# askerlee/segtran

Measured on AMD Instinct MI355X. Metric: train-step images/sec (cfg2, re-associated op order), higher is better.
Workload: dtype f32; 1 GPU; REFUGE fundus 2D, segtran eff-b4, translayers 3, layercompress 1,1,2,2, 512x512, bs 6/GPU; global_batch=6, per_gpu_batch=6, parallelism=dp1, step=fwd+BCE/Dice+bwd+allreduce+clip+BertAdam, op_order=re-associated, ranks=1

## Files before the change

include/segx.h:

```cpp
#ifndef SEGX_H
#define SEGX_H
#include <stdint.h>
#ifdef __cplusplus
extern "C" {
#endif

int segx_version(void);
int segx_last_error(char* buf, int buflen);

enum { SEGX_EPI_NONE = 0, SEGX_EPI_GELU = 1 ,
       SEGX_EPI_SWISH = 2 ,
       SEGX_EPI_RELU = 3  };
enum { SEGX_BIAS_NONE = 0, SEGX_BIAS_N = 1 , SEGX_BIAS_M = 2  };
enum { SEGX_ENGINE_F32 = 0, SEGX_ENGINE_BF16X6 = 1 };
enum { SEGX_ENGINE_SEL_DEFAULT = 0, SEGX_ENGINE_SEL_F32 = 1, SEGX_ENGINE_SEL_BF16X6 = 2 };
enum { SEGX_TILE_AUTO = 0, SEGX_TILE_128x128 = 1, SEGX_TILE_64x64 = 2, SEGX_TILE_128x32 = 3, SEGX_TILE_32x128 = 4, SEGX_TILE_64x128 = 5,
       SEGX_TILE_256x128 = 6, SEGX_TILE_WS128x128 = 7, SEGX_TILE_WS128x256 = 8, SEGX_TILE_WS64x256 = 9,
       SEGX_TILE_WS96x256 = 10, SEGX_TILE_WS256x96 = 11,
       SEGX_TILE_SKINNY_NT = 12   };
typedef struct {
    int32_t M, N, K, nb0, nb1;
    int64_t a_b0, a_b1, a_m, a_k;
    int64_t b_b0, b_b1, b_n, b_k;
    int64_t c_b0, c_b1, c_m;
// ... 163 lines not shown
int segx_set_rng_base(const uint64_t* base);
int segx_rng_advance(uint64_t* base, uint64_t span, void* stream);

enum {
    SEGX_KNOB_INTERP_VARIANT = 1,
    SEGX_KNOB_CONV_SMALL_POLICY = 2,
    SEGX_KNOB_BN_PATH = 3,
    SEGX_KNOB_ENGINE = 4,
    SEGX_KNOB_X6_LAUNCHES = 5,
    SEGX_KNOB_X6_VARIANT = 6,
    SEGX_KNOB_CONV_X6_WGRAD_ALL = 7,
    SEGX_KNOB_DW_STRIP_OUTPUTS = 8,
    SEGX_KNOB_WS_GRID = 9,
    SEGX_KNOB_TEAM_SPIN = 12,
    SEGX_KNOB_TEAM_DROP = 13,
    SEGX_KNOB_POOL_SLAB = 14,
    SEGX_KNOB_POOL_DSLIDE = 15,
    SEGX_KNOB_CONV_HALO = 16,
    SEGX_KNOB_CONV_HALO_MIN_TILES = 17,
    SEGX_KNOB_SKINNY_NT = 18,
    SEGX_KNOB_TILE_WALK = 19
};
#define SEGX_KNOB_X6_TERMS 20
int segx_tune(int knob, int value);
int segx_tune_get(int knob);
int segx_x3_launches(void);
int segx_interp_linear_fwd_axis2(const float* in, const float* base, float* out, int64_t outer, int n1_in, int n1_out, int n2_in, int n2_out,
                                 int64_t inner, void* stream);
int segx_interp_linear_bwd_axis2(const float* dout, float* din, int64_t outer, int n1_out, int n1_in, int n2_out, int n2_in, int64_t inner, void* stream);
int segx_interp_linear_fwd(const float* in, const float* base, float* out, int64_t planes, int d, int h, int w, int D, int H, int W,
                           void* stream);
int segx_interp_linear_fwd_axis(const float* in, const float* base, float* out, int64_t outer, int n_in, int n_out, int64_t inner,
                                float src_scale, void* stream);
int segx_resized_crop3d(const float* X, float* Y, int64_t planes, const int* geom, void* stream);
int segx_interp_linear_bwd(const float* dout, float* din, int64_t planes, int d, int h, int w, int D, int H, int W, void* stream);
int segx_axis_gather(const float* X, float* Y, int64_t planes, const int* geom, void* stream);
int segx_pixel_shuffle2(const float* X, float* Y, int64_t planes, int h, int w, int inverse, void* stream);
int segx_add_noise(const float* X, const float* noise, float* Y, int64_t n, float mu, float sigma, int nonzero_only, uint64_t seed, uint64_t offset,
                   void* stream);
int segx_resize2d(const float* X, float* Y, int64_t planes, int h, int w, int H, int W, int mode, int quantize, void* stream);
int segx_color_blend(const float* X, float* Y, int B, int64_t HW, int mode, const float* factor, const float* pivot, int quantize, void* stream);
int64_t segx_gray_mean_ws_floats(int B, int64_t HW);
int segx_gray_mean(const float* X, float* mean, float* ws, int B, int64_t HW, int quantize, void* stream);
int segx_normalize(const float* X, float* Y, int B, int C, int64_t HW, float scale, const float* mean, const float* std, void* stream);

int segx_interp_linear_bwd_axis(const float* dout, float* din, int64_t outer, int n_out, int n_in, int64_t inner, float src_scale,
// ... 91 lines not shown
```

segtran_amd/csrc/common.h:

```cpp
#pragma once
#include <hip/hip_runtime.h>
#include <stdint.h>
#include <stdio.h>
#include <stdarg.h>
#include <string.h>
#include <math.h>
#include <atomic>
#include "../../include/segx.h"

typedef float f32x16 __attribute__((ext_vector_type(16)));
typedef float f32x4 __attribute__((ext_vector_type(4)));

namespace segx {

inline char* err_buf() { static thread_local char buf[512] = {0}; return buf; }
inline int fail(int code, const char* fmt, ...) {
    va_list ap; va_start(ap, fmt); vsnprintf(err_buf(), 512, fmt, ap); va_end(ap); return code;
}
inline int check_launch(const char* what) {
    hipError_t e = hipGetLastError();
    if (e != hipSuccess) return fail((int)e, "%s: %s", what, hipGetErrorString(e));
    return 0;
}
#ifndef SEGX_MIN_WAVES_PER_SIMD
// ... 200 lines not shown
__device__ __forceinline__ float gelu_erf_grad(float x) {
    const float cdf = 0.5f * (1.0f + erff(x * 0.70710678118654752440f));
    const float pdf = 0.39894228040143267794f * __expf(-0.5f * x * x);
    return cdf + x * pdf;
}

#define SEGX_KNOB_TABLE(X)                                                                                                                                        \
    X(1, interp_variant, 0, 0, 2)                                                                  \
    X(2, conv_small_policy, 0, 0, 1)                          \
    X(3, bn_path, 0, 0, 2)                            \
    X(4, engine, SEGX_ENGINE_F32, SEGX_ENGINE_F32, SEGX_ENGINE_BF16X6)                                                                   \
    X(6, x6_variant, 0, 0, 7)                                      \
    X(7, conv_x6_wgrad_all, 0, 0, 2)                  \
    X(8, dw_strip_outputs, 8192, 256, 2147483647)                                                         \
    X(9, ws_grid, 256, 8, 4096)                                                                         \
    X(12, team_spin, (int)TEAM_SPIN_LIMIT, 32, 1 << 24)                                                     \
    X(13, team_drop, 0, 0, 4096)                      \
    X(14, pool_slab, 0, 0, 2)                         \
    X(15, pool_dslide, 1, 0, 1)                       \
    X(16, conv_halo, 1, 0, 1)                         \
    X(17, conv_halo_min_tiles, 256, 1, 1 << 24)         \
    X(18, skinny_nt, 1, 0, 1)                         \
    X(19, tile_walk, 1, 0, 1)                         \
    X(20, x6_terms, 6, 3, 6)
struct Knobs {
#define SEGX_KNOB_FIELD(id, field, def, lo, hi) std::atomic<int> field{def};
    SEGX_KNOB_TABLE(SEGX_KNOB_FIELD)
#undef SEGX_KNOB_FIELD
    std::atomic<int> x6_launches{0};
    std::atomic<int> x3_launches{0};
};
inline Knobs& knobs() { static Knobs k; return k; }
inline int kget(const std::atomic<int>& a) { return a.load(std::memory_order_relaxed); }
int halo_fwd_terms();

inline const uint64_t*& rng_base() { static const uint64_t* p = nullptr; return p; }

inline int ceil_div(int64_t a, int64_t b) { return (int)((a + b - 1) / b); }
__device__ __forceinline__ unsigned xcd_block(unsigned b, unsigned n) {
    const unsigned q = n >> 3, r = n & 7, xcd = b & 7, idx = b >> 3;
    return (xcd < r ? xcd * (q + 1) : r * (q + 1) + (xcd - r) * q) + idx;
}
__host__ __device__ inline int64_t i64min(int64_t a, int64_t b) { return a < b ? a : b; }
__host__ __device__ inline int64_t i64max(int64_t a, int64_t b) { return a > b ? a : b; }

struct FastDiv { unsigned d, magic; };
__host__ __device__ inline FastDiv make_fastdiv(int d) { FastDiv f; f.d = (unsigned)d; f.magic = d <= 1 ? 0u : (unsigned)(((1ull << 32) + d - 1) / d); return f; }
// ... 9 lines not shown
```

segtran_amd/csrc/mbconv_mid.hip:

```cpp
#include "common.h"
#include <initializer_list>

namespace segx {

constexpr int MID_BMAX = 6;

template <int NT> __device__ __forceinline__ void mid_guards(f32x4* pl, int H, int W4) {
    for (int r = threadIdx.x; r <= H; r += NT) pl[r * (W4 + 1)] = f32x4{0.f, 0.f, 0.f, 0.f};
}
__device__ __forceinline__ void mid_window(float (&e)[12], const f32x4* pl, int p, int r, int dr, int H, int W4) {
    const bool rok = (unsigned)(r + dr) < (unsigned)H;
    const f32x4* q = pl + (rok ? p + dr * (W4 + 1) : p);
    const f32x4 a = q[-1], m = q[0], z = q[1];
    e[0] = rok ? a.x : 0.f; e[1] = rok ? a.y : 0.f; e[2] = rok ? a.z : 0.f; e[3] = rok ? a.w : 0.f;
    e[4] = rok ? m.x : 0.f; e[5] = rok ? m.y : 0.f; e[6] = rok ? m.z : 0.f; e[7] = rok ? m.w : 0.f;
    e[8] = rok ? z.x : 0.f; e[9] = rok ? z.y : 0.f; e[10] = rok ? z.z : 0.f; e[11] = rok ? z.w : 0.f;
}
template <int NW, int KP>
__device__ __forceinline__ void mid_stats(f32x4 (&v)[MID_BMAX][KP], int B, float n, float* red, float& m, float& q) {
    float s = 0.f;
#pragma unroll
    for (int b = 0; b < MID_BMAX; ++b)
#pragma unroll
        for (int k = 0; k < KP; ++k) {
            if (b >= B) v[b][k] = f32x4{0.f, 0.f, 0.f, 0.f};
            s += (v[b][k].x + v[b][k].y) + (v[b][k].z + v[b][k].w);
        }
    m = block_sum<NW>(s, red) / n;
    q = 0.f;
#pragma unroll
    for (int b = 0; b < MID_BMAX; ++b)
#pragma unroll
        for (int k = 0; k < KP; ++k) {
            const float d0 = v[b][k].x - m, d1 = v[b][k].y - m, d2 = v[b][k].z - m, d3 = v[b][k].w - m;
            q += b < B ? (d0 * d0 + d1 * d1) + (d2 * d2 + d3 * d3) : 0.f;
        }
    q = block_sum<NW>(q, red);
}
__device__ __forceinline__ void mid_running(float* run_mean, float* run_var, int c, float momentum, float m, float q, float n) {
    if (run_mean) {
        run_mean[c] = (1.0f - momentum) * run_mean[c] + momentum * m;
        run_var[c] = (1.0f - momentum) * run_var[c] + momentum * (q / fmaxf(n - 1.0f, 1.0f));
    }
}

struct MidFwdArgs {
    const float* E; const float* w0; const float* b0; float* rm0; float* rv0; const float* Wdw; const float* w1; const float* b1; float* rm1; float* rv1;
    float* D; float* Y; float* psum; float* mean0; float* var0; float* mean1; float* var1;
    float mom0, eps0, mom1, eps1; int C, H, W4;
};
template <int KP, int K>
__global__ __launch_bounds__(256) SEGX_MIN_WAVES_PER_SIMD(KP == 1 ? 4 : 2) void mbconv_mid_fwd_kernel(MidFwdArgs g, int B) {
    constexpr int NT = 256, P = K / 2, S4 = NT * KP;
    __shared__ float red[4];
    __shared__ f32x4 plane[2 * S4 + 1];
    const int tl = threadIdx.x, c = blockIdx.x, C = g.C, H = g.H, W4 = g.W4;
    constexpr int64_t S = 4 * S4;
    unsigned off[KP]; int row[KP], pos[KP];
#pragma unroll
    for (int k = 0; k < KP; ++k) { const int j = tl + NT * k; off[k] = 16u * (unsigned)j; row[k] = j / W4; pos[k] = j + row[k] + 1; }
    mid_guards<NT>(plane, H, W4);
    f32x4 v[MID_BMAX][KP];
#pragma unroll
    for (int b = 0; b < MID_BMAX; ++b) {
        const ws_gptr xb = ws_uniform_base(g.E + ((int64_t)(b < B ? b : 0) * C + c) * S);
#pragma unroll
        for (int k = 0; k < KP; ++k) v[b][k] = ws_load<f32x4>(xb, off[k]);
    }
    __builtin_amdgcn_sched_barrier(0);
    float w[K * K];
#pragma unroll
    for (int i = 0; i < K * K; ++i) w[i] = g.Wdw[(int64_t)c * K * K + i];
    const float n = (float)B * (float)S;
    float m, q;
    mid_stats<4, KP>(v, B, n, red, m, q);
    float var = q / n;
    if (tl == 0) { g.mean0[c] = m; g.var0[c] = var; mid_running(g.rm0, g.rv0, c, g.mom0, m, q, n); }
    const float sc0 = rsqrtf(var + g.eps0) * g.w0[c], sh0 = g.b0[c] - m * sc0;
#pragma unroll
    for (int b = 0; b < MID_BMAX; ++b) {
        if (b >= B) break;
#pragma unroll
        for (int k = 0; k < KP; ++k) {
            f32x4 o;
            o.x = act_fwd(v[b][k].x * sc0 + sh0, ACT_SWISH); o.y = act_fwd(v[b][k].y * sc0 + sh0, ACT_SWISH);
            o.z = act_fwd(v[b][k].z * sc0 + sh0, ACT_SWISH); o.w = act_fwd(v[b][k].w * sc0 + sh0, ACT_SWISH);
            plane[pos[k]] = o;
        }
        __syncthreads();
        const ws_gptr_w db = ws_uniform_base_w(g.D + ((int64_t)b * C + c) * S);
#pragma unroll
        for (int k = 0; k < KP; ++k) {
            float acc[4] = {0.f, 0.f, 0.f, 0.f};
#pragma unroll
            for (int ky = 0; ky < K; ++ky) {
                float e[12];
                mid_window(e, plane, pos[k], row[k], ky - P, H, W4);
#pragma unroll
                for (int j = 0; j < 4; ++j)
#pragma unroll
                    for (int kx = 0; kx < K; ++kx) acc[j] += w[ky * K + kx] * e[4 + j + kx - P];
#pragma unroll
                for (int j = 0; j < 4; ++j) SEGX_PIN(acc[j]);
            }
            v[b][k] = f32x4{acc[0], acc[1], acc[2], acc[3]};
            ws_store<f32x4>(db, off[k], v[b][k]);
        }
        __syncthreads();
        __builtin_amdgcn_sched_barrier(0);
    }
    mid_stats<4, KP>(v, B, n, red, m, q);
    var = q / n;
    if (tl == 0) { g.mean1[c] = m; g.var1[c] = var; mid_running(g.rm1, g.rv1, c, g.mom1, m, q, n); }
    const float sc1 = rsqrtf(var + g.eps1) * g.w1[c], sh1 = g.b1[c] - m * sc1;
#pragma unroll
    for (int b = 0; b < MID_BMAX; ++b) {
        if (b >= B) break;
        const ws_gptr_w yb = ws_uniform_base_w(g.Y + ((int64_t)b * C + c) * S);
        float acc = 0.f;
#pragma unroll
        for (int k = 0; k < KP; ++k) {
            f32x4 o;
            o.x = act_fwd(v[b][k].x * sc1 + sh1, ACT_SWISH); o.y = act_fwd(v[b][k].y * sc1 + sh1, ACT_SWISH);
            o.z = act_fwd(v[b][k].z * sc1 + sh1, ACT_SWISH); o.w = act_fwd(v[b][k].w * sc1 + sh1, ACT_SWISH);
            ws_store<f32x4>(yb, off[k], o);
            acc += (o.x + o.y) + (o.z + o.w);
        }
        acc = block_sum<4>(acc, red);
        if (tl == 0) g.psum[(int64_t)b * C + c] = acc;
        __builtin_amdgcn_sched_barrier(0);
    }
}

__device__ __forceinline__ double wave_sum_d(double v) {
#pragma unroll
    for (int o = 32; o > 0; o >>= 1) v += __shfl_xor(v, o);
    return v;
}
template <int NW> __device__ __forceinline__ double block_sum_d(double v, double* red) {
    v = wave_sum_d(v);
    __syncthreads();
    if ((threadIdx.x & 63) == 0) red[threadIdx.x >> 6] = v;
    __syncthreads();
    double s = 0.0;
#pragma unroll
    for (int i = 0; i < NW; ++i) s += red[i];
    return s;
}

struct MidBwdArgs {
    const float* dY; const float* dpool; const float* D; const float* E;
    const float* mean0; const float* var0; const float* mean1; const float* var1;
    const float* w0; const float* b0; const float* w1; const float* b1; const float* Wdw;
    float* dE; float* dw0; float* db0; float* dw1; float* db1; float* dWdw;
    float inv_S, eps0, eps1; int C, H, W4;
};
template <int NT, int KP, int K, bool HL>
__global__ __launch_bounds__(NT) void mbconv_mid_bwd_kernel(MidBwdArgs g, int B) {
    constexpr int NW = NT / 64, P = K / 2, S4 = NT * KP, KK = K * K;
    __shared__ double red[NW];
    __shared__ double wred[NW][KK];
    __shared__ f32x4 plane[2 * S4 + 1];
    __shared__ f32x4 hl[HL ? MID_BMAX * S4 : 1];
    const int tl = threadIdx.x, c = blockIdx.x, C = g.C, H = g.H, W4 = g.W4;
    constexpr int64_t S = 4 * S4;
    unsigned off[KP]; int row[KP], pos[KP];
#pragma unroll
    for (int k = 0; k < KP; ++k) { const int j = tl + NT * k; off[k] = 16u * (unsigned)j; row[k] = j / W4; pos[k] = j + row[k] + 1; }
    mid_guards<NT>(plane, H, W4);
    f32x4 h[MID_BMAX][KP], d[MID_BMAX][KP];
    auto hget = [&](int b, int k) -> f32x4 { if constexpr (HL) return hl[(b * KP + k) * NT + tl]; else return h[b][k]; };
    auto hput = [&](int b, int k, f32x4 x) { if constexpr (HL) hl[(b * KP + k) * NT + tl] = x; else h[b][k] = x; };
#pragma unroll
    for (int b = 0; b < MID_BMAX; ++b) {
        const int64_t po = ((int64_t)(b < B ? b : 0) * C + c) * S;
        const ws_gptr xb = ws_uniform_base(g.D + po), gb = ws_uniform_base(g.dY + po);
#pragma unroll
        for (int k = 0; k < KP; ++k) { h[b][k] = ws_load<f32x4>(xb, off[k]); d[b][k] = ws_load<f32x4>(gb, off[k]); }
    }
    f32x4 ev[KP];
    {
        const ws_gptr eb = ws_uniform_base(g.E + (int64_t)c * S);
#pragma unroll
        for (int k = 0; k < KP; ++k) ev[k] = ws_load<f32x4>(eb, off[k]);
    }
    __builtin_amdgcn_sched_barrier(0);
    float w[KK], dwa[KK];
#pragma unroll
    for (int i = 0; i < KK; ++i) { w[i] = g.Wdw[(int64_t)c * KK + i]; dwa[i] = 0.f; }
    const double inv_n = 1.0 / ((double)B * (double)S);
    const float rstd1 = rsqrtf(g.var1[c] + g.eps1), m1 = g.mean1[c], w1c = g.w1[c], b1c = g.b1[c];
    double a = 0.0, q = 0.0;
#pragma unroll
    for (int b = 0; b < MID_BMAX; ++b) {
        const bool bok = b < B;
        const float dp = g.dpool[(bok ? b : 0) * C + c] * g.inv_S;
#pragma unroll
        for (int k = 0; k < KP; ++k) {
            const f32x4 xv = h[b][k], gv = d[b][k];
            f32x4 hh, dd;
            hh.x = (xv.x - m1) * rstd1; hh.y = (xv.y - m1) * rstd1; hh.z = (xv.z - m1) * rstd1; hh.w = (xv.w - m1) * rstd1;
            dd.x = (gv.x + dp) * act_grad(hh.x * w1c + b1c, ACT_SWISH); dd.y = (gv.y + dp) * act_grad(hh.y * w1c + b1c, ACT_SWISH);
            dd.z = (gv.z + dp) * act_grad(hh.z * w1c + b1c, ACT_SWISH); dd.w = (gv.w + dp) * act_grad(hh.w * w1c + b1c, ACT_SWISH);
            if (!bok) { dd = f32x4{0.f, 0.f, 0.f, 0.f}; hh = dd; }
            hput(b, k, hh); d[b][k] = dd;
            a += (double)((dd.x + dd.y) + (dd.z + dd.w)); q += (double)((dd.x * hh.x + dd.y * hh.y) + (dd.z * hh.z + dd.w * hh.w));
        }
        __builtin_amdgcn_sched_barrier(0);
    }
    a = block_sum_d<NW>(a, red); q = block_sum_d<NW>(q, red);
    if (tl == 0) { g.db1[c] = (float)a; g.dw1[c] = (float)q; }
    const double k1 = a * inv_n, k2 = q * inv_n, sc1 = (double)(w1c * rstd1);
    const float k1f = (float)k1, k2f = (float)k2, sc1f = w1c * rstd1;
    const float rstd0 = rsqrtf(g.var0[c] + g.eps0), m0 = g.mean0[c], sc0 = rstd0 * g.w0[c], sh0 = g.b0[c] - m0 * sc0;
    double a0 = 0.0, q0 = 0.0;
#pragma unroll
    for (int b = 0; b < MID_BMAX; ++b) {
        if (b >= B) break;
#pragma unroll
        for (int k = 0; k < KP; ++k) {
            const f32x4 hh = hget(b, k);
            f32x4 o;
            if constexpr (HL) {
                o.x = (float)(sc1 * ((double)d[b][k].x - k1 - (double)hh.x * k2)); o.y = (float)(sc1 * ((double)d[b][k].y - k1 - (double)hh.y * k2));
                o.z = (float)(sc1 * ((double)d[b][k].z - k1 - (double)hh.z * k2)); o.w = (float)(sc1 * ((double)d[b][k].w - k1 - (double)hh.w * k2));
            } else {
                o.x = sc1f * (d[b][k].x - k1f - hh.x * k2f); o.y = sc1f * (d[b][k].y - k1f - hh.y * k2f);
                o.z = sc1f * (d[b][k].z - k1f - hh.z * k2f); o.w = sc1f * (d[b][k].w - k1f - hh.w * k2f);
            }
            plane[pos[k]] = o;
        }
        __syncthreads();
#pragma unroll
        for (int k = 0; k < KP; ++k) {
            const f32x4 xv = ev[k];
            const float u[4] = {xv.x * sc0 + sh0, xv.y * sc0 + sh0, xv.z * sc0 + sh0, xv.w * sc0 + sh0};
            float ep[4], de[4] = {0.f, 0.f, 0.f, 0.f};
#pragma unroll
            for (int i = 0; i < 4; ++i) ep[i] = act_fwd(u[i], ACT_SWISH);
#pragma unroll
            for (int ry = -P; ry <= P; ++ry) {
                float e[12];
                mid_window(e, plane, pos[k], row[k], ry, H, W4);
#pragma unroll
                for (int rx = -P; rx <= P; ++rx) {
                    const int t = (P - ry) * K + (P - rx);
#pragma unroll
                    for (int i = 0; i < 4; ++i) {
                        de[i] = __builtin_fmaf(w[t], e[4 + i + rx], de[i]); dwa[t] = __builtin_fmaf(ep[i], e[4 + i + rx], dwa[t]);
                        SEGX_PIN(de[i]); SEGX_PIN(dwa[t]);
                    }
                }
                __builtin_amdgcn_sched_barrier(0);
            }
            f32x4 hh, dd;
            hh.x = (xv.x - m0) * rstd0; hh.y = (xv.y - m0) * rstd0; hh.z = (xv.z - m0) * rstd0; hh.w = (xv.w - m0) * rstd0;
            dd.x = de[0] * act_grad(u[0], ACT_SWISH); dd.y = de[1] * act_grad(u[1], ACT_SWISH);
            dd.z = de[2] * act_grad(u[2], ACT_SWISH); dd.w = de[3] * act_grad(u[3], ACT_SWISH);
            hput(b, k, hh); d[b][k] = dd;
            a0 += (double)((dd.x + dd.y) + (dd.z + dd.w)); q0 += (double)((dd.x * hh.x + dd.y * hh.y) + (dd.z * hh.z + dd.w * hh.w));
        }
        if (b + 1 < MID_BMAX) {
            const ws_gptr eb = ws_uniform_base(g.E + ((int64_t)(b + 1 < B ? b + 1 : b) * C + c) * S);
#pragma unroll
            for (int k = 0; k < KP; ++k) ev[k] = ws_load<f32x4>(eb, off[k]);
        }
        __syncthreads();
        __builtin_amdgcn_sched_barrier(0);
    }
    a0 = block_sum_d<NW>(a0, red); q0 = block_sum_d<NW>(q0, red);
    if (tl == 0) { g.db0[c] = (float)a0; g.dw0[c] = (float)q0; }
    const float j1 = (float)(a0 * inv_n), j2 = (float)(q0 * inv_n);
#pragma unroll
    for (int b = 0; b < MID_BMAX; ++b) {
        if (b >= B) break;
        const ws_gptr_w ob = ws_uniform_base_w(g.dE + ((int64_t)b * C + c) * S);
#pragma unroll
        for (int k = 0; k < KP; ++k) {
            const f32x4 hh = hget(b, k);
            f32x4 o;
            o.x = sc0 * (d[b][k].x - j1 - hh.x * j2); o.y = sc0 * (d[b][k].y - j1 - hh.y * j2);
            o.z = sc0 * (d[b][k].z - j1 - hh.z * j2); o.w = sc0 * (d[b][k].w - j1 - hh.w * j2);
            ws_store<f32x4>(ob, off[k], o);
        }
        __builtin_amdgcn_sched_barrier(0);
    }
#pragma unroll
    for (int i = 0; i < KK; ++i) { const double s = wave_sum_d((double)dwa[i]); if ((tl & 63) == 0) wred[tl >> 6][i] = s; }
    __syncthreads();
    if (tl < KK) {
        double s = 0.0;
#pragma unroll
        for (int i = 0; i < NW; ++i) s += wred[i][tl];
        g.dWdw[(int64_t)c * KK + tl] = (float)s;
    }
}

static inline bool mid_serves(int B, int C, int H, int W, int k) {
    return B >= 1 && B <= MID_BMAX && C >= 1 && H >= 1 && W >= 4 && W % 4 == 0 && (k == 3 || k == 5) && ((int64_t)H * W == 1024 || (int64_t)H * W == 4096);
}
static inline bool mid_aligned(std::initializer_list<const void*> ps) {
    for (const void* p : ps) if (reinterpret_cast<uintptr_t>(p) & 15) return false;
    return true;
}

}

using namespace segx;
#define SEGX_STREAM hipStream_t stream = (hipStream_t)stream_

extern "C" int segx_mbconv_mid_ok(int B, int C, int H, int W, int k) { return mid_serves(B, C, H, W, k) ? 1 : 0; }

extern "C" int segx_mbconv_mid_fwd(const float* E, const float* w0, const float* b0, float* run_mean0, float* run_var0, const float* Wdw, const float* w1, const float* b1,
                                   float* run_mean1, float* run_var1, float* D, float* Y, float* psum, float* mean0, float* var0, float* mean1, float* var1,
                                   float momentum0, float eps0, float momentum1, float eps1, int B, int C, int H, int W, int k, void* stream_) {
    SEGX_STREAM; SEGX_REQUIRE(E && w0 && b0 && Wdw && w1 && b1 && D && Y && psum && mean0 && var0 && mean1 && var1 && (!run_mean0 == !run_var0) && (!run_mean1 == !run_var1),
                              "segx_mbconv_mid_fwd: bad args");
    SEGX_REQUIRE(mid_serves(B, C, H, W, k), "segx_mbconv_mid_fwd: shape not served (segx_mbconv_mid_ok == 0)");
    SEGX_REQUIRE(mid_aligned({E, D, Y}), "segx_mbconv_mid_fwd: tensors must be 16-byte aligned");
    const MidFwdArgs g{E, w0, b0, run_mean0, run_var0, Wdw, w1, b1, run_mean1, run_var1, D, Y, psum, mean0, var0, mean1, var1, momentum0, eps0, momentum1, eps1, C, H, W / 4};
#define SEGX_MID_F(KP, K) hipLaunchKernelGGL((mbconv_mid_fwd_kernel<KP, K>), dim3((unsigned)C), dim3(256), 0, stream, g, B)
    if (H * W == 4096) { if (k == 3) SEGX_MID_F(4, 3); else SEGX_MID_F(4, 5); }
    else { if (k == 3) SEGX_MID_F(1, 3); else SEGX_MID_F(1, 5); }
#undef SEGX_MID_F
    return check_launch("segx_mbconv_mid_fwd");
}

extern "C" int segx_mbconv_mid_bwd(const float* dY, const float* dpool, const float* D, const float* E, const float* mean0, const float* var0, const float* mean1,
                                   const float* var1, const float* w0, const float* b0, const float* w1, const float* b1, const float* Wdw,
                                   float* dE, float* dw0, float* db0, float* dw1, float* db1, float* dWdw, float inv_S, float eps0, float eps1,
                                   int B, int C, int H, int W, int k, void* stream_) {
    SEGX_STREAM; SEGX_REQUIRE(dY && dpool && D && E && mean0 && var0 && mean1 && var1 && w0 && b0 && w1 && b1 && Wdw && dE && dw0 && db0 && dw1 && db1 && dWdw, "segx_mbconv_mid_bwd: bad args");
    SEGX_REQUIRE(mid_serves(B, C, H, W, k), "segx_mbconv_mid_bwd: shape not served (segx_mbconv_mid_ok == 0)");
    SEGX_REQUIRE(mid_aligned({dY, D, E, dE}), "segx_mbconv_mid_bwd: tensors must be 16-byte aligned");
    const MidBwdArgs g{dY, dpool, D, E, mean0, var0, mean1, var1, w0, b0, w1, b1, Wdw, dE, dw0, db0, dw1, db1, dWdw, inv_S, eps0, eps1, C, H, W / 4};
#define SEGX_MID_B(NT, KP, K, HL) hipLaunchKernelGGL((mbconv_mid_bwd_kernel<NT, KP, K, HL>), dim3((unsigned)C), dim3(NT), 0, stream, g, B)
    if (H * W == 4096) { if (k == 3) SEGX_MID_B(1024, 1, 3, true); else SEGX_MID_B(512, 2, 5, true); }
    else { if (k == 3) SEGX_MID_B(256, 1, 3, false); else SEGX_MID_B(256, 1, 5, false); }
#undef SEGX_MID_B
    return check_launch("segx_mbconv_mid_bwd");
}
```

segtran_amd/segx.py:

```python
import contextlib
import ctypes
import enum
import os
import torch

_HERE = os.path.dirname(os.path.abspath(__file__))
LIB_PATH = os.path.join(_HERE, 'lib', 'libsegx.so')

c_f = ctypes.c_float
c_i = ctypes.c_int32
c_l = ctypes.c_int64
c_u = ctypes.c_uint64
c_p = ctypes.c_void_p


class GemmDesc(ctypes.Structure):
    _fields_ = [('M', c_i), ('N', c_i), ('K', c_i), ('nb0', c_i), ('nb1', c_i),
                ('a_b0', c_l), ('a_b1', c_l), ('a_m', c_l), ('a_k', c_l),
                ('b_b0', c_l), ('b_b1', c_l), ('b_n', c_l), ('b_k', c_l),
                ('c_b0', c_l), ('c_b1', c_l), ('c_m', c_l),
                ('alpha', c_f), ('epilogue', c_i), ('bias_mode', c_i), ('bias_b1', c_l),
                ('bias', c_p), ('aux', c_p), ('gmax', c_p),
                ('dropout_p', c_f), ('seed', c_u), ('offset', c_u),
                ('splitk', c_i), ('workspace', c_p), ('tile', c_i), ('bias_b0', c_l), ('batch_reduce', c_i), ('engine', c_i),
# ... 7 lines not shown


class Knob(enum.IntEnum):
    INTERP_VARIANT = 1
    CONV_SMALL_POLICY = 2
    BN_PATH = 3
    ENGINE = 4
    X6_LAUNCHES = 5
    X6_VARIANT = 6
    CONV_X6_WGRAD_ALL = 7
    DW_STRIP_OUTPUTS = 8
    WS_GRID = 9
    TEAM_SPIN = 12
    TEAM_DROP = 13
    POOL_SLAB = 14
    POOL_DSLIDE = 15
    CONV_HALO = 16
    CONV_HALO_MIN_TILES = 17
    SKINNY_NT = 18
    TILE_WALK = 19


Knob.X6_TERMS = 20


def knob_id(name):
    v = getattr(Knob, name.upper(), None)
    if not isinstance(v, int) or name.upper().startswith('_'):
        raise KeyError(name)
    return v


def _ptr(t):
    return None if t is None else t.data_ptr()


_raw_stream = getattr(torch._C, '_cuda_getCurrentRawStream', None)


class SegxLib:
    def __init__(self, path=LIB_PATH):
        if not os.path.exists(path):
            raise RuntimeError('libsegx not built: %s is missing '
                               '(run `python -c "import __graft_entry__ as g; g.build()"`)' % path)
        self.path = path
        self.c = ctypes.CDLL(path)
# ... 751 lines not shown
```

Baseline: 96.58 images/s.

## Make mbconv mid kernels persistent with next-channel prefetch and zero guard rows

Result: no change. 96.82 images/s, median of 6 (+0.2%).

```diff
diff --git a/include/segx.h b/include/segx.h
--- a/include/segx.h
+++ b/include/segx.h
@@ -209,6 +209,7 @@
     SEGX_KNOB_TILE_WALK = 19
 };
 #define SEGX_KNOB_X6_TERMS 20
+#define SEGX_KNOB_MID_GRID 22
 int segx_tune(int knob, int value);
 int segx_tune_get(int knob);
 int segx_x3_launches(void);
diff --git a/segtran_amd/csrc/common.h b/segtran_amd/csrc/common.h
--- a/segtran_amd/csrc/common.h
+++ b/segtran_amd/csrc/common.h
@@ -246,7 +246,8 @@
     X(17, conv_halo_min_tiles, 256, 1, 1 << 24)         \
     X(18, skinny_nt, 1, 0, 1)                         \
     X(19, tile_walk, 1, 0, 1)                         \
-    X(20, x6_terms, 6, 3, 6)
+    X(20, x6_terms, 6, 3, 6)                          \
+    X(22, mid_grid, 0, 0, 1 << 20)
 struct Knobs {
 #define SEGX_KNOB_FIELD(id, field, def, lo, hi) std::atomic<int> field{def};
     SEGX_KNOB_TABLE(SEGX_KNOB_FIELD)
diff --git a/segtran_amd/csrc/mbconv_mid.hip b/segtran_amd/csrc/mbconv_mid.hip
--- a/segtran_amd/csrc/mbconv_mid.hip
+++ b/segtran_amd/csrc/mbconv_mid.hip
@@ -1,20 +1,30 @@
 #include "common.h"
 #include <initializer_list>
+#include <map>
+#include <mutex>
+#include <utility>
 
 namespace segx {
 
 constexpr int MID_BMAX = 6;
 
-template <int NT> __device__ __forceinline__ void mid_guards(f32x4* pl, int H, int W4) {
-    for (int r = threadIdx.x; r <= H; r += NT) pl[r * (W4 + 1)] = f32x4{0.f, 0.f, 0.f, 0.f};
-}
-__device__ __forceinline__ void mid_window(float (&e)[12], const f32x4* pl, int p, int r, int dr, int H, int W4) {
-    const bool rok = (unsigned)(r + dr) < (unsigned)H;
-    const f32x4* q = pl + (rok ? p + dr * (W4 + 1) : p);
-    const f32x4 a = q[-1], m = q[0], z = q[1];
-    e[0] = rok ? a.x : 0.f; e[1] = rok ? a.y : 0.f; e[2] = rok ? a.z : 0.f; e[3] = rok ? a.w : 0.f;
-    e[4] = rok ? m.x : 0.f; e[5] = rok ? m.y : 0.f; e[6] = rok ? m.z : 0.f; e[7] = rok ? m.w : 0.f;
-    e[8] = rok ? z.x : 0.f; e[9] = rok ? z.y : 0.f; e[10] = rok ? z.z : 0.f; e[11] = rok ? z.w : 0.f;
+template <int NT, int PR> __device__ __forceinline__ void mid_guards(f32x4* pl, int H, int W4) {
+    if constexpr (PR > 0) { for (int i = threadIdx.x; i < (H + 2 * PR) * (W4 + 1) + 1; i += NT) pl[i] = f32x4{0.f, 0.f, 0.f, 0.f}; }
+    else { for (int r = threadIdx.x; r <= H; r += NT) pl[r * (W4 + 1)] = f32x4{0.f, 0.f, 0.f, 0.f}; }
+}
+template <bool GR> __device__ __forceinline__ void mid_window(float (&e)[12], const f32x4* pl, int p, int r, int dr, int H, int W4) {
+    if constexpr (GR) {
+        const f32x4* q = pl + p + dr * (W4 + 1);
+        const f32x4 a = q[-1], m = q[0], z = q[1];
+        e[0] = a.x; e[1] = a.y; e[2] = a.z; e[3] = a.w; e[4] = m.x; e[5] = m.y; e[6] = m.z; e[7] = m.w; e[8] = z.x; e[9] = z.y; e[10] = z.z; e[11] = z.w;
+    } else {
+        const bool rok = (unsigned)(r + dr) < (unsigned)H;
+        const f32x4* q = pl + (rok ? p + dr * (W4 + 1) : p);
+        const f32x4 a = q[-1], m = q[0], z = q[1];
+        e[0] = rok ? a.x : 0.f; e[1] = rok ? a.y : 0.f; e[2] = rok ? a.z : 0.f; e[3] = rok ? a.w : 0.f;
+        e[4] = rok ? m.x : 0.f; e[5] = rok ? m.y : 0.f; e[6] = rok ? m.z : 0.f; e[7] = rok ? m.w : 0.f;
+        e[8] = rok ? z.x : 0.f; e[9] = rok ? z.y : 0.f; e[10] = rok ? z.z : 0.f; e[11] = rok ? z.w : 0.f;
+    }
 }
 template <int NW, int KP>
 __device__ __forceinline__ void mid_stats(f32x4 (&v)[MID_BMAX][KP], int B, float n, float* red, float& m, float& q) {
@@ -49,86 +59,96 @@
     float* D; float* Y; float* psum; float* mean0; float* var0; float* mean1; float* var1;
     float mom0, eps0, mom1, eps1; int C, H, W4;
 };
-template <int KP, int K>
+template <int KP, int K, bool GR>
 __global__ __launch_bounds__(256) SEGX_MIN_WAVES_PER_SIMD(KP == 1 ? 4 : 2) void mbconv_mid_fwd_kernel(MidFwdArgs g, int B) {
-    constexpr int NT = 256, P = K / 2, S4 = NT * KP;
+    constexpr int NT = 256, P = K / 2, S4 = NT * KP, PR = GR ? P : 0;
     __shared__ float red[4];
     __shared__ f32x4 plane[2 * S4 + 1];
-    const int tl = threadIdx.x, c = blockIdx.x, C = g.C, H = g.H, W4 = g.W4;
+    const int tl = threadIdx.x, C = g.C, H = g.H, W4 = g.W4, G = (int)gridDim.x;
     constexpr int64_t S = 4 * S4;
     unsigned off[KP]; int row[KP], pos[KP];
 #pragma unroll
-    for (int k = 0; k < KP; ++k) { const int j = tl + NT * k; off[k] = 16u * (unsigned)j; row[k] = j / W4; pos[k] = j + row[k] + 1; }
-    mid_guards<NT>(plane, H, W4);
+    for (int k = 0; k < KP; ++k) { const int j = tl + NT * k; off[k] = 16u * (unsigned)j; row[k] = j / W4; pos[k] = j + row[k] + 1 + PR * (W4 + 1); }
+    mid_guards<NT, PR>(plane, H, W4);
     f32x4 v[MID_BMAX][KP];
 #pragma unroll
     for (int b = 0; b < MID_BMAX; ++b) {
-        const ws_gptr xb = ws_uniform_base(g.E + ((int64_t)(b < B ? b : 0) * C + c) * S);
+        const ws_gptr xb = ws_uniform_base(g.E + ((int64_t)(b < B ? b : 0) * C + blockIdx.x) * S);
 #pragma unroll
         for (int k = 0; k < KP; ++k) v[b][k] = ws_load<f32x4>(xb, off[k]);
     }
-    __builtin_amdgcn_sched_barrier(0);
-    float w[K * K];
-#pragma unroll
-    for (int i = 0; i < K * K; ++i) w[i] = g.Wdw[(int64_t)c * K * K + i];
-    const float n = (float)B * (float)S;
-    float m, q;
-    mid_stats<4, KP>(v, B, n, red, m, q);
-    float var = q / n;
-    if (tl == 0) { g.mean0[c] = m; g.var0[c] = var; mid_running(g.rm0, g.rv0, c, g.mom0, m, q, n); }
-    const float sc0 = rsqrtf(var + g.eps0) * g.w0[c], sh0 = g.b0[c] - m * sc0;
-#pragma unroll
-    for (int b = 0; b < MID_BMAX; ++b) {
-        if (b >= B) break;
-#pragma unroll
-        for (int k = 0; k < KP; ++k) {
-            f32x4 o;
-            o.x = act_fwd(v[b][k].x * sc0 + sh0, ACT_SWISH); o.y = act_fwd(v[b][k].y * sc0 + sh0, ACT_SWISH);
-            o.z = act_fwd(v[b][k].z * sc0 + sh0, ACT_SWISH); o.w = act_fwd(v[b][k].w * sc0 + sh0, ACT_SWISH);
-            plane[pos[k]] = o;
-        }
-        __syncthreads();
-        const ws_gptr_w db = ws_uniform_base_w(g.D + ((int64_t)b * C + c) * S);
-#pragma unroll
-        for (int k = 0; k < KP; ++k) {
-            float acc[4] = {0.f, 0.f, 0.f, 0.f};
-#pragma unroll
-            for (int ky = 0; ky < K; ++ky) {
-                float e[12];
-                mid_window(e, plane, pos[k], row[k], ky - P, H, W4);
-#pragma unroll
-                for (int j = 0; j < 4; ++j)
-#pragma unroll
-                    for (int kx = 0; kx < K; ++kx) acc[j] += w[ky * K + kx] * e[4 + j + kx - P];
-#pragma unroll
-                for (int j = 0; j < 4; ++j) SEGX_PIN(acc[j]);
-            }
-            v[b][k] = f32x4{acc[0], acc[1], acc[2], acc[3]};
-            ws_store<f32x4>(db, off[k], v[b][k]);
-        }
-        __syncthreads();
+    for (int c = blockIdx.x; c < C; c += G) {
+        const bool more = c + G < C;
         __builtin_amdgcn_sched_barrier(0);
-    }
-    mid_stats<4, KP>(v, B, n, red, m, q);
-    var = q / n;
-    if (tl == 0) { g.mean1[c] = m; g.var1[c] = var; mid_running(g.rm1, g.rv1, c, g.mom1, m, q, n); }
-    const float sc1 = rsqrtf(var + g.eps1) * g.w1[c], sh1 = g.b1[c] - m * sc1;
-#pragma unroll
-    for (int b = 0; b < MID_BMAX; ++b) {
-        if (b >= B) break;
-        const ws_gptr_w yb = ws_uniform_base_w(g.Y + ((int64_t)b * C + c) * S);
-        float acc = 0.f;
-#pragma unroll
-        for (int k = 0; k < KP; ++k) {
-            f32x4 o;
-            o.x = act_fwd(v[b][k].x * sc1 + sh1, ACT_SWISH); o.y = act_fwd(v[b][k].y * sc1 + sh1, ACT_SWISH);
-            o.z = act_fwd(v[b][k].z * sc1 + sh1, ACT_SWISH); o.w = act_fwd(v[b][k].w * sc1 + sh1, ACT_SWISH);
-            ws_store<f32x4>(yb, off[k], o);
-            acc += (o.x + o.y) + (o.z + o.w);
-        }
-        acc = block_sum<4>(acc, red);
-        if (tl == 0) g.psum[(int64_t)b * C + c] = acc;
-        __builtin_amdgcn_sched_barrier(0);
+        float w[K * K];
+#pragma unroll
+        for (int i = 0; i < K * K; ++i) w[i] = g.Wdw[(int64_t)c * K * K + i];
+        const float n = (float)B * (float)S;
+        float m, q;
+        mid_stats<4, KP>(v, B, n, red, m, q);
+        float var = q / n;
+        if (tl == 0) { g.mean0[c] = m; g.var0[c] = var; mid_running(g.rm0, g.rv0, c, g.mom0, m, q, n); }
+        const float sc0 = rsqrtf(var + g.eps0) * g.w0[c], sh0 = g.b0[c] - m * sc0;
+#pragma unroll
+        for (int b = 0; b < MID_BMAX; ++b) {
+            if (b >= B) break;
+#pragma unroll
+            for (int k = 0; k < KP; ++k) {
+                f32x4 o;
+                o.x = act_fwd(v[b][k].x * sc0 + sh0, ACT_SWISH); o.y = act_fwd(v[b][k].y * sc0 + sh0, ACT_SWISH);
+                o.z = act_fwd(v[b][k].z * sc0 + sh0, ACT_SWISH); o.w = act_fwd(v[b][k].w * sc0 + sh0, ACT_SWISH);
+                plane[pos[k]] = o;
+            }
+            __syncthreads();
+            const ws_gptr_w db = ws_uniform_base_w(g.D + ((int64_t)b * C + c) * S);
+#pragma unroll
+            for (int k = 0; k < KP; ++k) {
+                float acc[4] = {0.f, 0.f, 0.f, 0.f};
+                int pk = pos[k]; SEGX_PIN(pk);
+#pragma unroll
+                for (int ky = 0; ky < K; ++ky) {
+#pragma clang fp contract(on)
+                    float e[12];
+                    mid_window<GR>(e, plane, pk, row[k], ky - P, H, W4);
+#pragma unroll
+                    for (int j = 0; j < 4; ++j)
+#pragma unroll
+                        for (int kx = 0; kx < K; ++kx) acc[j] += w[ky * K + kx] * e[4 + j + kx - P];
+#pragma unroll
+                    for (int j = 0; j < 4; ++j) SEGX_PIN(acc[j]);
+                }
+                v[b][k] = f32x4{acc[0], acc[1], acc[2], acc[3]};
+                ws_store<f32x4>(db, off[k], v[b][k]);
+            }
+            __syncthreads();
+            __builtin_amdgcn_sched_barrier(0);
+        }
+        mid_stats<4, KP>(v, B, n, red, m, q);
+        var = q / n;
+        if (tl == 0) { g.mean1[c] = m; g.var1[c] = var; mid_running(g.rm1, g.rv1, c, g.mom1, m, q, n); }
+        const float sc1 = rsqrtf(var + g.eps1) * g.w1[c], sh1 = g.b1[c] - m * sc1;
+#pragma unroll
+        for (int b = 0; b < MID_BMAX; ++b) {
+            if (b >= B) break;
+            const ws_gptr_w yb = ws_uniform_base_w(g.Y + ((int64_t)b * C + c) * S);
+            float acc = 0.f;
+#pragma unroll
+            for (int k = 0; k < KP; ++k) {
+                f32x4 o;
+                o.x = act_fwd(v[b][k].x * sc1 + sh1, ACT_SWISH); o.y = act_fwd(v[b][k].y * sc1 + sh1, ACT_SWISH);
+                o.z = act_fwd(v[b][k].z * sc1 + sh1, ACT_SWISH); o.w = act_fwd(v[b][k].w * sc1 + sh1, ACT_SWISH);
+                ws_store<f32x4>(yb, off[k], o);
+                acc += (o.x + o.y) + (o.z + o.w);
+            }
+            if (more) {
+                const ws_gptr xb = ws_uniform_base(g.E + ((int64_t)b * C + c + G) * S);
+#pragma unroll
+                for (int k = 0; k < KP; ++k) v[b][k] = ws_load<f32x4>(xb, off[k]);
+            }
+            acc = block_sum<4>(acc, red);
+            if (tl == 0) g.psum[(int64_t)b * C + c] = acc;
+            __builtin_amdgcn_sched_barrier(0);
+        }
     }
 }
 
@@ -148,6 +168,7 @@
     return s;
 }
 
+constexpr bool mid_bwd_walks(int NT) { return NT == 512; }
 struct MidBwdArgs {
     const float* dY; const float* dpool; const float* D; const float* E;
     const float* mean0; const float* var0; const float* mean1; const float* var1;
@@ -155,145 +176,162 @@
     float* dE; float* dw0; float* db0; float* dw1; float* db1; float* dWdw;
     float inv_S, eps0, eps1; int C, H, W4;
 };
-template <int NT, int KP, int K, bool HL>
+template <int NT, int KP, int K, bool HL, bool GR>
 __global__ __launch_bounds__(NT) void mbconv_mid_bwd_kernel(MidBwdArgs g, int B) {
-    constexpr int NW = NT / 64, P = K / 2, S4 = NT * KP, KK = K * K;
+    constexpr int NW = NT / 64, P = K / 2, S4 = NT * KP, KK = K * K, PR = GR ? P : 0;
+    constexpr bool WALK = mid_bwd_walks(NT), DS = HL && GR;
     __shared__ double red[NW];
     __shared__ double wred[NW][KK];
     __shared__ f32x4 plane[2 * S4 + 1];
     __shared__ f32x4 hl[HL ? MID_BMAX * S4 : 1];
-    const int tl = threadIdx.x, c = blockIdx.x, C = g.C, H = g.H, W4 = g.W4;
+    const int tl = threadIdx.x, C = g.C, H = g.H, W4 = g.W4, G = (int)gridDim.x;
     constexpr int64_t S = 4 * S4;
     unsigned off[KP]; int row[KP], pos[KP];
 #pragma unroll
-    for (int k = 0; k < KP; ++k) { const int j = tl + NT * k; off[k] = 16u * (unsigned)j; row[k] = j / W4; pos[k] = j + row[k] + 1; }
-    mid_guards<NT>(plane, H, W4);
+    for (int k = 0; k < KP; ++k) { const int j = tl + NT * k; off[k] = 16u * (unsigned)j; row[k] = j / W4; pos[k] = j + row[k] + 1 + PR * (W4 + 1); }
+    mid_guards<NT, PR>(plane, H, W4);
     f32x4 h[MID_BMAX][KP], d[MID_BMAX][KP];
     auto hget = [&](int b, int k) -> f32x4 { if constexpr (HL) return hl[(b * KP + k) * NT + tl]; else return h[b][k]; };
     auto hput = [&](int b, int k, f32x4 x) { if constexpr (HL) hl[(b * KP + k) * NT + tl] = x; else h[b][k] = x; };
 #pragma unroll
     for (int b = 0; b < MID_BMAX; ++b) {
-        const int64_t po = ((int64_t)(b < B ? b : 0) * C + c) * S;
+        const int64_t po = ((int64_t)(b < B ? b : 0) * C + blockIdx.x) * S;
         const ws_gptr xb = ws_uniform_base(g.D + po), gb = ws_uniform_base(g.dY + po);
 #pragma unroll
         for (int k = 0; k < KP; ++k) { h[b][k] = ws_load<f32x4>(xb, off[k]); d[b][k] = ws_load<f32x4>(gb, off[k]); }
     }
     f32x4 ev[KP];
     {
-        const ws_gptr eb = ws_uniform_base(g.E + (int64_t)c * S);
+        const ws_gptr eb = ws_uniform_base(g.E + (int64_t)blockIdx.x * S);
 #pragma unroll
         for (int k = 0; k < KP; ++k) ev[k] = ws_load<f32x4>(eb, off[k]);
     }
-    __builtin_amdgcn_sched_barrier(0);
-    float w[KK], dwa[KK];
-#pragma unroll
-    for (int i = 0; i < KK; ++i) { w[i] = g.Wdw[(int64_t)c * KK + i]; dwa[i] = 0.f; }
-    const double inv_n = 1.0 / ((double)B * (double)S);
-    const float rstd1 = rsqrtf(g.var1[c] + g.eps1), m1 = g.mean1[c], w1c = g.w1[c], b1c = g.b1[c];
-    double a = 0.0, q = 0.0;
-#pragma unroll
-    for (int b = 0; b < MID_BMAX; ++b) {
-        const bool bok = b < B;
-        const float dp = g.dpool[(bok ? b : 0) * C + c] * g.inv_S;
-#pragma unroll
-        for (int k = 0; k < KP; ++k) {
-            const f32x4 xv = h[b][k], gv = d[b][k];
-            f32x4 hh, dd;
-            hh.x = (xv.x - m1) * rstd1; hh.y = (xv.y - m1) * rstd1; hh.z = (xv.z - m1) * rstd1; hh.w = (xv.w - m1) * rstd1;
-            dd.x = (gv.x + dp) * act_grad(hh.x * w1c + b1c, ACT_SWISH); dd.y = (gv.y + dp) * act_grad(hh.y * w1c + b1c, ACT_SWISH);
-            dd.z = (gv.z + dp) * act_grad(hh.z * w1c + b1c, ACT_SWISH); dd.w = (gv.w + dp) * act_grad(hh.w * w1c + b1c, ACT_SWISH);
-            if (!bok) { dd = f32x4{0.f, 0.f, 0.f, 0.f}; hh = dd; }
-            hput(b, k, hh); d[b][k] = dd;
-            a += (double)((dd.x + dd.y) + (dd.z + dd.w)); q += (double)((dd.x * hh.x + dd.y * hh.y) + (dd.z * hh.z + dd.w * hh.w));
-        }
+    int c = blockIdx.x;
+    do {
+        const bool more = WALK && c + G < C;
         __builtin_amdgcn_sched_barrier(0);
-    }
-    a = block_sum_d<NW>(a, red); q = block_sum_d<NW>(q, red);
-    if (tl == 0) { g.db1[c] = (float)a; g.dw1[c] = (float)q; }
-    const double k1 = a * inv_n, k2 = q * inv_n, sc1 = (double)(w1c * rstd1);
-    const float k1f = (float)k1, k2f = (float)k2, sc1f = w1c * rstd1;
-    const float rstd0 = rsqrtf(g.var0[c] + g.eps0), m0 = g.mean0[c], sc0 = rstd0 * g.w0[c], sh0 = g.b0[c] - m0 * sc0;
-    double a0 = 0.0, q0 = 0.0;
-#pragma unroll
-    for (int b = 0; b < MID_BMAX; ++b) {
-        if (b >= B) break;
-#pragma unroll
-        for (int k = 0; k < KP; ++k) {
-            const f32x4 hh = hget(b, k);
-            f32x4 o;
-            if constexpr (HL) {
-                o.x = (float)(sc1 * ((double)d[b][k].x - k1 - (double)hh.x * k2)); o.y = (float)(sc1 * ((double)d[b][k].y - k1 - (double)hh.y * k2));
-                o.z = (float)(sc1 * ((double)d[b][k].z - k1 - (double)hh.z * k2)); o.w = (float)(sc1 * ((double)d[b][k].w - k1 - (double)hh.w * k2));
-            } else {
-                o.x = sc1f * (d[b][k].x - k1f - hh.x * k2f); o.y = sc1f * (d[b][k].y - k1f - hh.y * k2f);
-                o.z = sc1f * (d[b][k].z - k1f - hh.z * k2f); o.w = sc1f * (d[b][k].w - k1f - hh.w * k2f);
-            }
-            plane[pos[k]] = o;
-        }
+        float w[KK], dwa[KK];
+#pragma unroll
+        for (int i = 0; i < KK; ++i) { w[i] = g.Wdw[(int64_t)c * KK + i]; dwa[i] = 0.f; }
+        const double inv_n = 1.0 / ((double)B * (double)S);
+        const float rstd1 = rsqrtf(g.var1[c] + g.eps1), m1 = g.mean1[c], w1c = g.w1[c], b1c = g.b1[c];
+        double a = 0.0, q = 0.0;
+#pragma unroll
+        for (int b = 0; b < MID_BMAX; ++b) {
+            const bool bok = b < B;
+            const float dp = g.dpool[(bok ? b : 0) * C + c] * g.inv_S;
+#pragma unroll
+            for (int k = 0; k < KP; ++k) {
+                const f32x4 xv = h[b][k], gv = d[b][k];
+                f32x4 hh, dd;
+                hh.x = (xv.x - m1) * rstd1; hh.y = (xv.y - m1) * rstd1; hh.z = (xv.z - m1) * rstd1; hh.w = (xv.w - m1) * rstd1;
+                dd.x = (gv.x + dp) * act_grad(hh.x * w1c + b1c, ACT_SWISH); dd.y = (gv.y + dp) * act_grad(hh.y * w1c + b1c, ACT_SWISH);
+                dd.z = (gv.z + dp) * act_grad(hh.z * w1c + b1c, ACT_SWISH); dd.w = (gv.w + dp) * act_grad(hh.w * w1c + b1c, ACT_SWISH);
+                if (!bok) { dd = f32x4{0.f, 0.f, 0.f, 0.f}; hh = dd; }
+                hput(b, k, hh); d[b][k] = dd;
+                a += (double)((dd.x + dd.y) + (dd.z + dd.w)); q += (double)((dd.x * hh.x + dd.y * hh.y) + (dd.z * hh.z + dd.w * hh.w));
+            }
+            __builtin_amdgcn_sched_barrier(0);
+        }
+        a = block_sum_d<NW>(a, red); q = block_sum_d<NW>(q, red);
+        if (tl == 0) { g.db1[c] = (float)a; g.dw1[c] = (float)q; }
+        const double k1 = a * inv_n, k2 = q * inv_n, sc1 = (double)(w1c * rstd1);
+        const float k1f = (float)k1, k2f = (float)k2, sc1f = w1c * rstd1;
+        const float rstd0 = rsqrtf(g.var0[c] + g.eps0), m0 = g.mean0[c], sc0 = rstd0 * g.w0[c], sh0 = g.b0[c] - m0 * sc0;
+        double a0 = 0.0, q0 = 0.0;
+#pragma unroll
+        for (int b = 0; b < MID_BMAX; ++b) {
+            if (b >= B) break;
+#pragma unroll
+            for (int k = 0; k < KP; ++k) {
+                const f32x4 hh = hget(b, k);
+                f32x4 o;
+                if constexpr (HL) {
+                    o.x = (float)(sc1 * ((double)d[b][k].x - k1 - (double)hh.x * k2)); o.y = (float)(sc1 * ((double)d[b][k].y - k1 - (double)hh.y * k2));
+                    o.z = (float)(sc1 * ((double)d[b][k].z - k1 - (double)hh.z * k2)); o.w = (float)(sc1 * ((double)d[b][k].w - k1 - (double)hh.w * k2));
+                } else {
+                    o.x = sc1f * (d[b][k].x - k1f - hh.x * k2f); o.y = sc1f * (d[b][k].y - k1f - hh.y * k2f);
+                    o.z = sc1f * (d[b][k].z - k1f - hh.z * k2f); o.w = sc1f * (d[b][k].w - k1f - hh.w * k2f);
+                }
+                plane[pos[k]] = o;
+            }
+            __syncthreads();
+#pragma unroll
+            for (int k = 0; k < KP; ++k) {
+                const f32x4 xv = ev[k];
+                const float u[4] = {xv.x * sc0 + sh0, xv.y * sc0 + sh0, xv.z * sc0 + sh0, xv.w * sc0 + sh0};
+                float ep[4], de[4] = {0.f, 0.f, 0.f, 0.f};
+#pragma unroll
+                for (int i = 0; i < 4; ++i) ep[i] = act_fwd(u[i], ACT_SWISH);
+#pragma unroll
+                for (int ry = -P; ry <= P; ++ry) {
+                    float e[12];
+                    mid_window<GR>(e, plane, pos[k], row[k], ry, H, W4);
+#pragma unroll
+                    for (int rx = -P; rx <= P; ++rx) {
+                        const int t = (P - ry) * K + (P - rx);
+#pragma unroll
+                        for (int i = 0; i < 4; ++i) {
+                            de[i] = __builtin_fmaf(w[t], e[4 + i + rx], de[i]); dwa[t] = __builtin_fmaf(ep[i], e[4 + i + rx], dwa[t]);
+                            SEGX_PIN(de[i]); SEGX_PIN(dwa[t]);
+                        }
+                    }
+                    __builtin_amdgcn_sched_barrier(0);
+                }
+                f32x4 hh, dd;
+                hh.x = (xv.x - m0) * rstd0; hh.y = (xv.y - m0) * rstd0; hh.z = (xv.z - m0) * rstd0; hh.w = (xv.w - m0) * rstd0;
+                dd.x = de[0] * act_grad(u[0], ACT_SWISH); dd.y = de[1] * act_grad(u[1], ACT_SWISH);
+                dd.z = de[2] * act_grad(u[2], ACT_SWISH); dd.w = de[3] * act_grad(u[3], ACT_SWISH);
+                hput(b, k, hh); d[b][k] = dd;
+                a0 += (double)((dd.x + dd.y) + (dd.z + dd.w)); q0 += (double)((dd.x * hh.x + dd.y * hh.y) + (dd.z * hh.z + dd.w * hh.w));
+            }
+            const bool last = b + 1 >= B;
+            if (!last || more) {
+                const ws_gptr eb = ws_uniform_base(g.E + ((int64_t)(last ? 0 : b + 1) * C + (last ? c + G : c)) * S);
+#pragma unroll
+                for (int k = 0; k < KP; ++k) ev[k] = ws_load<f32x4>(eb, off[k]);
+            }
+            if constexpr (DS) if (more) {
+                const ws_gptr xb = ws_uniform_base(g.D + ((int64_t)b * C + c + G) * S);
+#pragma unroll
+                for (int k = 0; k < KP; ++k) h[b][k] = ws_load<f32x4>(xb, off[k]);
+            }
+            __syncthreads();
+            __builtin_amdgcn_sched_barrier(0);
+        }
+        a0 = block_sum_d<NW>(a0, red); q0 = block_sum_d<NW>(q0, red);
+        if (tl == 0) { g.db0[c] = (float)a0; g.dw0[c] = (float)q0; }
+        const float j1 = (float)(a0 * inv_n), j2 = (float)(q0 * inv_n);
+#pragma unroll
+        for (int b = 0; b < MID_BMAX; ++b) {
+            if (b >= B) break;
+            const ws_gptr_w ob = ws_uniform_base_w(g.dE + ((int64_t)b * C + c) * S);
+#pragma unroll
+            for (int k = 0; k < KP; ++k) {
+                const f32x4 hh = hget(b, k);
+                f32x4 o;
+                o.x = sc0 * (d[b][k].x - j1 - hh.x * j2); o.y = sc0 * (d[b][k].y - j1 - hh.y * j2);
+                o.z = sc0 * (d[b][k].z - j1 - hh.z * j2); o.w = sc0 * (d[b][k].w - j1 - hh.w * j2);
+                ws_store<f32x4>(ob, off[k], o);
+            }
+            if (more) {
+                const int64_t po = ((int64_t)b * C + c + G) * S;
+                const ws_gptr xb = ws_uniform_base(g.D + po), gb = ws_uniform_base(g.dY + po);
+#pragma unroll
+                for (int k = 0; k < KP; ++k) { if constexpr (!DS) h[b][k] = ws_load<f32x4>(xb, off[k]); d[b][k] = ws_load<f32x4>(gb, off[k]); }
+            }
+            __builtin_amdgcn_sched_barrier(0);
+        }
+#pragma unroll
+        for (int i = 0; i < KK; ++i) { const double s = wave_sum_d((double)dwa[i]); if ((tl & 63) == 0) wred[tl >> 6][i] = s; }
         __syncthreads();
-#pragma unroll
-        for (int k = 0; k < KP; ++k) {
-            const f32x4 xv = ev[k];
-            const float u[4] = {xv.x * sc0 + sh0, xv.y * sc0 + sh0, xv.z * sc0 + sh0, xv.w * sc0 + sh0};
-            float ep[4], de[4] = {0.f, 0.f, 0.f, 0.f};
-#pragma unroll
-            for (int i = 0; i < 4; ++i) ep[i] = act_fwd(u[i], ACT_SWISH);
-#pragma unroll
-            for (int ry = -P; ry <= P; ++ry) {
-                float e[12];
-                mid_window(e, plane, pos[k], row[k], ry, H, W4);
-#pragma unroll
-                for (int rx = -P; rx <= P; ++rx) {
-                    const int t = (P - ry) * K + (P - rx);
-#pragma unroll
-                    for (int i = 0; i < 4; ++i) {
-                        de[i] = __builtin_fmaf(w[t], e[4 + i + rx], de[i]); dwa[t] = __builtin_fmaf(ep[i], e[4 + i + rx], dwa[t]);
-                        SEGX_PIN(de[i]); SEGX_PIN(dwa[t]);
-                    }
-                }
-                __builtin_amdgcn_sched_barrier(0);
-            }
-            f32x4 hh, dd;
-            hh.x = (xv.x - m0) * rstd0; hh.y = (xv.y - m0) * rstd0; hh.z = (xv.z - m0) * rstd0; hh.w = (xv.w - m0) * rstd0;
-            dd.x = de[0] * act_grad(u[0], ACT_SWISH); dd.y = de[1] * act_grad(u[1], ACT_SWISH);
-            dd.z = de[2] * act_grad(u[2], ACT_SWISH); dd.w = de[3] * act_grad(u[3], ACT_SWISH);
-            hput(b, k, hh); d[b][k] = dd;
-            a0 += (double)((dd.x + dd.y) + (dd.z + dd.w)); q0 += (double)((dd.x * hh.x + dd.y * hh.y) + (dd.z * hh.z + dd.w * hh.w));
-        }
-        if (b + 1 < MID_BMAX) {
-            const ws_gptr eb = ws_uniform_base(g.E + ((int64_t)(b + 1 < B ? b + 1 : b) * C + c) * S);
-#pragma unroll
-            for (int k = 0; k < KP; ++k) ev[k] = ws_load<f32x4>(eb, off[k]);
-        }
-        __syncthreads();
-        __builtin_amdgcn_sched_barrier(0);
-    }
-    a0 = block_sum_d<NW>(a0, red); q0 = block_sum_d<NW>(q0, red);
-    if (tl == 0) { g.db0[c] = (float)a0; g.dw0[c] = (float)q0; }
-    const float j1 = (float)(a0 * inv_n), j2 = (float)(q0 * inv_n);
-#pragma unroll
-    for (int b = 0; b < MID_BMAX; ++b) {
-        if (b >= B) break;
-        const ws_gptr_w ob = ws_uniform_base_w(g.dE + ((int64_t)b * C + c) * S);
-#pragma unroll
-        for (int k = 0; k < KP; ++k) {
-            const f32x4 hh = hget(b, k);
-            f32x4 o;
-            o.x = sc0 * (d[b][k].x - j1 - hh.x * j2); o.y = sc0 * (d[b][k].y - j1 - hh.y * j2);
-            o.z = sc0 * (d[b][k].z - j1 - hh.z * j2); o.w = sc0 * (d[b][k].w - j1 - hh.w * j2);
-            ws_store<f32x4>(ob, off[k], o);
-        }
-        __builtin_amdgcn_sched_barrier(0);
-    }
-#pragma unroll
-    for (int i = 0; i < KK; ++i) { const double s = wave_sum_d((double)dwa[i]); if ((tl & 63) == 0) wred[tl >> 6][i] = s; }
-    __syncthreads();
-    if (tl < KK) {
-        double s = 0.0;
-#pragma unroll
-        for (int i = 0; i < NW; ++i) s += wred[i][tl];
-        g.dWdw[(int64_t)c * KK + tl] = (float)s;
-    }
+        if (tl < KK) {
+            double s = 0.0;
+#pragma unroll
+            for (int i = 0; i < NW; ++i) s += wred[i][tl];
+            g.dWdw[(int64_t)c * KK + tl] = (float)s;
+        }
+    } while (WALK && (c += G) < C);
 }
 
 static inline bool mid_serves(int B, int C, int H, int W, int k) {
@@ -302,6 +340,27 @@
 static inline bool mid_aligned(std::initializer_list<const void*> ps) {
     for (const void* p : ps) if (reinterpret_cast<uintptr_t>(p) & 15) return false;
     return true;
+}
+static inline bool mid_guard_rows(int H, int W, int k) { return (int64_t)(H + 2 * (k / 2)) * (W / 4 + 1) <= 2 * (int64_t)H * (W / 4); }
+static int mid_grid(const void* kernel, int threads, int C) {
+    const int v = kget(knobs().mid_grid);
+    if (v > 0) return v < C ? v : C;
+    static std::mutex mu; static std::map<std::pair<const void*, int>, int> seen;
+    int dev = 0;
+    if (hipGetDevice(&dev) != hipSuccess) { (void)hipGetLastError(); return C; }
+    int slots;
+    {
+        std::lock_guard<std::mutex> lk(mu);
+        auto it = seen.find({kernel, dev});
+        if (it == seen.end()) {
+            int cus = 0, per = 0;
+            if (hipDeviceGetAttribute(&cus, hipDeviceAttributeMultiprocessorCount, dev) != hipSuccess) { (void)hipGetLastError(); cus = 0; }
+            if (hipOccupancyMaxActiveBlocksPerMultiprocessor(&per, kernel, threads, 0) != hipSuccess) { (void)hipGetLastError(); per = 0; }
+            it = seen.emplace(std::make_pair(kernel, dev), cus > 0 && per > 0 ? cus * per : 0).first;
+        }
+        slots = it->second;
+    }
+    return slots > 0 && slots < C ? slots : C;
 }
 
 }
@@ -319,10 +378,13 @@
     SEGX_REQUIRE(mid_serves(B, C, H, W, k), "segx_mbconv_mid_fwd: shape not served (segx_mbconv_mid_ok == 0)");
     SEGX_REQUIRE(mid_aligned({E, D, Y}), "segx_mbconv_mid_fwd: tensors must be 16-byte aligned");
     const MidFwdArgs g{E, w0, b0, run_mean0, run_var0, Wdw, w1, b1, run_mean1, run_var1, D, Y, psum, mean0, var0, mean1, var1, momentum0, eps0, momentum1, eps1, C, H, W / 4};
-#define SEGX_MID_F(KP, K) hipLaunchKernelGGL((mbconv_mid_fwd_kernel<KP, K>), dim3((unsigned)C), dim3(256), 0, stream, g, B)
+    const bool gr = mid_guard_rows(H, W, k);
+#define SEGX_MID_F1(KP, K, GR) hipLaunchKernelGGL((mbconv_mid_fwd_kernel<KP, K, GR>), dim3((unsigned)mid_grid((const void*)mbconv_mid_fwd_kernel<KP, K, GR>, 256, C)), dim3(256), 0, stream, g, B)
+#define SEGX_MID_F(KP, K) do { if (gr) SEGX_MID_F1(KP, K, true); else SEGX_MID_F1(KP, K, false); } while (0)
     if (H * W == 4096) { if (k == 3) SEGX_MID_F(4, 3); else SEGX_MID_F(4, 5); }
     else { if (k == 3) SEGX_MID_F(1, 3); else SEGX_MID_F(1, 5); }
 #undef SEGX_MID_F
+#undef SEGX_MID_F1
     return check_launch("segx_mbconv_mid_fwd");
 }
 
@@ -334,9 +396,12 @@
     SEGX_REQUIRE(mid_serves(B, C, H, W, k), "segx_mbconv_mid_bwd: shape not served (segx_mbconv_mid_ok == 0)");
     SEGX_REQUIRE(mid_aligned({dY, D, E, dE}), "segx_mbconv_mid_bwd: tensors must be 16-byte aligned");
     const MidBwdArgs g{dY, dpool, D, E, mean0, var0, mean1, var1, w0, b0, w1, b1, Wdw, dE, dw0, db0, dw1, db1, dWdw, inv_S, eps0, eps1, C, H, W / 4};
-#define SEGX_MID_B(NT, KP, K, HL) hipLaunchKernelGGL((mbconv_mid_bwd_kernel<NT, KP, K, HL>), dim3((unsigned)C), dim3(NT), 0, stream, g, B)
+    const bool gr = mid_guard_rows(H, W, k);
+#define SEGX_MID_B1(NT, KP, K, HL, GR) hipLaunchKernelGGL((mbconv_mid_bwd_kernel<NT, KP, K, HL, GR>), dim3((unsigned)(mid_bwd_walks(NT) ? mid_grid((const void*)mbconv_mid_bwd_kernel<NT, KP, K, HL, GR>, NT, C) : C)), dim3(NT), 0, stream, g, B)
+#define SEGX_MID_B(NT, KP, K, HL) do { if (gr) SEGX_MID_B1(NT, KP, K, HL, true); else SEGX_MID_B1(NT, KP, K, HL, false); } while (0)
     if (H * W == 4096) { if (k == 3) SEGX_MID_B(1024, 1, 3, true); else SEGX_MID_B(512, 2, 5, true); }
     else { if (k == 3) SEGX_MID_B(256, 1, 3, false); else SEGX_MID_B(256, 1, 5, false); }
 #undef SEGX_MID_B
+#undef SEGX_MID_B1
     return check_launch("segx_mbconv_mid_bwd");
 }
diff --git a/segtran_amd/segx.py b/segtran_amd/segx.py
--- a/segtran_amd/segx.py
+++ b/segtran_amd/segx.py
@@ -53,6 +53,7 @@
 
 
 Knob.X6_TERMS = 20
+Knob.MID_GRID = 22
 
 
 def knob_id(name):
```
